# wenz116/lang2seg

Hardware: AMD Instinct MI355X
Metric: train images/sec (cycle loss on), 600×1000 input, at 1/2/4/8 MI355X (higher is better)
Workload: dtype bf16; 1 GPU; train_cycle.sh step: ResNet-101 C4 + 7 spatial dynamic filters + att2in2 cycle loss, 600x1000 image, 20-token expression (V=3349), 12000->2000 proposals, 256 RoIs, per-GPU batch 1; variant=cycle, parallelism=dp1

## Files before the change

### lang2seg_amd/csrc/roi.hip

```cpp
#include "common.h"
#include "roi_sample.h"
#include "../../include/lang2seg_hip.h"

namespace {

__global__ void rpn_decode_kernel(const float* __restrict__ heads, int ldh, const float* __restrict__ base, int H, int W, int A,
                                  int fs, float im_h, float im_w, float* prob, float* boxes, float* scores) {
  const int n = H * W * A;
  for (int i = blockIdx.x * blockDim.x + threadIdx.x; i < n; i += gridDim.x * blockDim.x) {
    const int a = i % A, pix = i / A, w = pix % W, h = pix / W;
    const float* hr = heads + (long)pix * ldh;
    const float bg = hr[a], fg = hr[A + a];
    const float m = fmaxf(bg, fg);
    const float e0 = expf(bg - m), e1 = expf(fg - m);
    const float s = e0 + e1;
    prob[(long)pix * 2 * A + a] = e0 / s;
    prob[(long)pix * 2 * A + A + a] = e1 / s;
    scores[i] = e1 / s;
    const float ax1 = base[a * 4 + 0] + (float)(w * fs), ay1 = base[a * 4 + 1] + (float)(h * fs);
    const float ax2 = base[a * 4 + 2] + (float)(w * fs), ay2 = base[a * 4 + 3] + (float)(h * fs);
    const float aw = ax2 - ax1 + 1.0f, ah = ay2 - ay1 + 1.0f;
    const float cx = ax1 + 0.5f * aw, cy = ay1 + 0.5f * ah;
    const float* d = hr + 2 * A + a * 4;
    const float pcx = d[0] * aw + cx, pcy = d[1] * ah + cy;
    const float pw = expf(d[2]) * aw, ph = expf(d[3]) * ah;
    float x1 = pcx - 0.5f * pw, y1 = pcy - 0.5f * ph, x2 = pcx + 0.5f * pw, y2 = pcy + 0.5f * ph;
    x1 = fminf(fmaxf(x1, 0.f), im_w - 1.f); y1 = fminf(fmaxf(y1, 0.f), im_h - 1.f);
    x2 = fminf(fmaxf(x2, 0.f), im_w - 1.f); y2 = fminf(fmaxf(y2, 0.f), im_h - 1.f);
    *(float4*)(boxes + (long)i * 4) = make_float4(x1, y1, x2, y2);
  }
}

__device__ __forceinline__ uint64_t sort_key(float s, int idx) {
  uint32_t u = __float_as_uint(s);
  u = (u & 0x80000000u) ? ~u : (u | 0x80000000u);
  return ((uint64_t)u << 32) | (uint32_t)(0xFFFFFFFFu - (uint32_t)idx);
}
__device__ __forceinline__ unsigned int okey(float s) { unsigned int u = __float_as_uint(s); return (u & 0x80000000u) ? ~u : (u | 0x80000000u); }
struct RsWs { unsigned int* kA; int* iA; unsigned int* kB; int* iB; int* hist; };
__device__ __host__ __forceinline__ RsWs rs_ws(int* ws, int n) {
  RsWs w; w.kA = (unsigned int*)ws; w.iA = ws + n; w.kB = (unsigned int*)(ws + 2 * n); w.iB = ws + 3 * n; w.hist = ws + 4 * n;
  return w;
}
__global__ __launch_bounds__(256) void rs_hist0_kernel(const float* scores, int n, int nblk, int* hist) {
  __shared__ int h[256];
  const int t = threadIdx.x, b = blockIdx.x;
  h[t] = 0;
  __syncthreads();
  const int i = b * 256 + t;
  if (i < n) atomicAdd(&h[(~okey(scores[i])) & 255], 1);
  __syncthreads();
  hist[b * 256 + t] = h[t];
#pragma unroll
  for (int p = 1; p < 4; ++p) hist[(p * nblk + b) * 256 + t] = 0;
}
template <int PASS>
__global__ __launch_bounds__(256) void rs_pass_kernel(const float* __restrict__ scores, const float* __restrict__ boxes, const unsigned int* __restrict__ kin,
                                                      const int* __restrict__ iin, unsigned int* __restrict__ kout, int* __restrict__ iout, int n, int nblk,
                                                      int* __restrict__ hist, int k, float* __restrict__ sboxes, float* __restrict__ sscores, int* __restrict__ sidx) {
  __shared__ int tot[256], base[256], wcnt[4][256];
  const int t = threadIdx.x, b = blockIdx.x, lane = t & 63, wave = t >> 6;
  const int i = b * 256 + t;
  unsigned int key = 0; int idx = 0;
  const bool valid = i < n;
  if (valid) {
    if (PASS == 0) { key = ~okey(scores[i]); idx = i; } else { key = kin[i]; idx = iin[i]; }
  }
  const int d = (int)((key >> (8 * PASS)) & 255u);
  __shared__ int ptot[4][256], pbef[4][256];
  {
    const int q = t & 63, g = t >> 6;
    const int4* hp4 = (const int4*)(hist + (long)PASS * nblk * 256) + q;
    int4 tv = make_int4(0, 0, 0, 0), bv = make_int4(0, 0, 0, 0);
    for (int b0 = g; b0 < nblk; b0 += 64) {
      int4 v[16];
#pragma unroll
      for (int u = 0; u < 16; ++u) v[u] = (b0 + 4 * u < nblk) ? hp4[(long)(b0 + 4 * u) * 64] : make_int4(0, 0, 0, 0);
#pragma unroll
      for (int u = 0; u < 16; ++u) {
        tv.x += v[u].x; tv.y += v[u].y; tv.z += v[u].z; tv.w += v[u].w;
        if (b0 + 4 * u < b) { bv.x += v[u].x; bv.y += v[u].y; bv.z += v[u].z; bv.w += v[u].w; }
      }
    }
    *(int4*)&ptot[g][4 * q] = tv; *(int4*)&pbef[g][4 * q] = bv;
  }
  __syncthreads();
  const int total = ptot[0][t] + ptot[1][t] + ptot[2][t] + ptot[3][t];
  const int before = pbef[0][t] + pbef[1][t] + pbef[2][t] + pbef[3][t];
#pragma unroll
  for (int w = 0; w < 4; ++w) wcnt[w][t] = 0;
  int incl = total;
#pragma unroll
  for (int o = 1; o < 64; o <<= 1) { const int x = __shfl_up(incl, o); if (lane >= o) incl += x; }
  if (lane == 63) tot[wave] = incl;
  __syncthreads();
  for (int w = 0; w < wave; ++w) incl += tot[w];
  base[t] = incl - total + before;
  unsigned long long same = valid ? ~0ull : 0ull;
#pragma unroll
  for (int bit = 0; bit < 8; ++bit) {
    const unsigned long long bal = __ballot(valid && ((d >> bit) & 1));
    same &= ((d >> bit) & 1) ? bal : ~bal;
  }
  same &= __ballot(valid);
  const int below = __popcll(same & ((1ull << lane) - 1ull));
  if (valid && below == 0) wcnt[wave][d] = __popcll(same);
  __syncthreads();
  if (valid) {
    int rank = below;
    for (int w = 0; w < wave; ++w) rank += wcnt[w][d];
    const int pos = base[d] + rank;
    if (PASS < 3) {
      kout[pos] = key; iout[pos] = idx;
      atomicAdd(&hist[((long)(PASS + 1) * nblk + (pos >> 8)) * 256 + ((key >> (8 * (PASS + 1))) & 255u)], 1);
    } else if (pos < k) {
      sidx[pos] = idx; sscores[pos] = scores[idx];
      *(float4*)(sboxes + (long)pos * 4) = *(const float4*)(boxes + (long)idx * 4);
    }
  }
}

__device__ __forceinline__ bool nms_hit(const float4& a, float aarea, const float4& b, float barea, float thr, int cmp) {
  const float xx1 = fmaxf(a.x, b.x), yy1 = fmaxf(a.y, b.y), xx2 = fminf(a.z, b.z), yy2 = fminf(a.w, b.w);
  const float w = fmaxf(0.f, xx2 - xx1 + 1.f), h = fmaxf(0.f, yy2 - yy1 + 1.f);
  const float inter = w * h;
  const float uni = aarea + barea - inter;
  const float q = thr * uni;
  if (inter < q * (1.f - 0x1p-18f)) return false;
  if (inter > q * (1.f + 0x1p-18f)) return true;
  const float ovr = inter / uni;
  return cmp ? (ovr > thr) : (ovr >= thr);
}
#ifdef L2S_TOOLS
__device__ long long nms_dbg[16];
#define NMS_T() ((long long)__builtin_readcyclecounter())
#else
#define NMS_T() 0ll
#endif
constexpr int NMS_SB = 64;
constexpr int NMS_LAG = 6;
constexpr int NMS_RING = 16;
constexpr int NMS_SLOT = NMS_LAG + 2;
__global__ __launch_bounds__(256) void nms_mask_kernel(const float* __restrict__ boxes, int n, float thr, int cmp, int row0, int sbw, uint64_t* mask,
                                                       unsigned long long* carry_base, const int* __restrict__ keep, const int* nk_p, int max_keep,
                                                       unsigned long long* carry_all, int carry_words) {
  const int wv = threadIdx.x >> 6, lane = threadIdx.x & 63;
  const int cbk = blockIdx.x * 4 + wv;
  int nk = 0;
  if (row0 > 0) { nk = *nk_p; if (nk < 0 || nk >= max_keep) return; }
  else if (blockIdx.x == 0 && blockIdx.y == 0) for (int i = threadIdx.x; i < carry_words; i += 256) carry_all[i] = 0ull;
  const bool diag = (int)blockIdx.y < sbw;
  const int rb = blockIdx.y;
  const bool active = cbk < sbw && (diag ? cbk <= rb : ((int)blockIdx.y - sbw) * 64 < nk);
  __shared__ float4 cbox_s[4][64];
  __shared__ float carea_s[4][64];
  float4* cbox = cbox_s[wv]; float* carea = carea_s[wv];
  const int cj = row0 + cbk * 64 + lane;
  const float4 cbv = (active && cj < n) ? *(const float4*)(boxes + (long)cj * 4) : make_float4(0, 0, -1, -1);
  cbox[lane] = cbv;
  carea[lane] = (cbv.z - cbv.x + 1.f) * (cbv.w - cbv.y + 1.f);
  __syncthreads();
  if (!active) return;
  unsigned long long* carry = carry_base;
  const int csize = min(64, n - row0 - cbk * 64);
  if (diag) {
    const int ri = row0 + rb * 64 + lane;
    if (ri >= n) return;
    const float4 a = *(const float4*)(boxes + (long)ri * 4);
    const float aarea = (a.z - a.x + 1.f) * (a.w - a.y + 1.f);
    uint64_t t = 0;
    if (rb == cbk) {
      for (int j = 0; j < lane; ++j)
        if (nms_hit(cbox[j], carea[j], a, aarea, thr, cmp)) t |= 1ull << j;
    } else {
      for (int j = 0; j < 64; ++j)
        if (nms_hit(cbox[j], carea[j], a, aarea, thr, cmp)) t |= 1ull << j;
    }
    mask[(long)(rb * sbw + cbk) * 64 + lane] = t;
    return;
  }
  const int ki = ((int)blockIdx.y - sbw) * 64 + lane;
  uint64_t t = 0;
  if (ki < nk) {
    const int ri = keep[ki];
    const float4 a = *(const float4*)(boxes + (long)ri * 4);
    const float aarea = (a.z - a.x + 1.f) * (a.w - a.y + 1.f);
    for (int j = 0; j < csize; ++j)
      if (nms_hit(a, aarea, cbox[j], carea[j], thr, cmp)) t |= 1ull << j;
  }
  unsigned int lo = (unsigned int)t, hi = (unsigned int)(t >> 32);
#pragma unroll
  for (int off = 32; off; off >>= 1) { lo |= __shfl_xor(lo, off); hi |= __shfl_xor(hi, off); }
  if (lane == 0 && (lo | hi)) atomicOr(&carry[cbk], ((unsigned long long)hi << 32) | lo);
}
__global__ __launch_bounds__(1024) void nms_reduce_kernel(const uint64_t* __restrict__ mask, int n, int cb, int max_keep, int* keep, int* num_out,
                                                          int row0, const unsigned long long* __restrict__ carry) {
  constexpr int LAG = NMS_LAG, SLOT = NMS_SLOT, NBULK = 15;
  extern __shared__ unsigned long long slots[];
  __shared__ int kdone_sh, stop_sh;
  __shared__ int ready_sh[NMS_SB];
  unsigned long long* ksh = slots + (size_t)NMS_RING * SLOT * 64;
  unsigned long long* csh = ksh + cb;
  const int tid = threadIdx.x, lane = tid & 63, wave = __builtin_amdgcn_readfirstlane(tid >> 6);
  int nk0 = 0;
  if (row0 > 0) { nk0 = *num_out; if (nk0 < 0 || nk0 >= max_keep) return; }
  for (int c = tid; c < cb; c += 1024) { ksh[c] = 0ull; csh[c] = carry ? carry[c] : 0ull; ready_sh[c] = 0; }
  if (tid == 0) { kdone_sh = 0; stop_sh = 0; }
  __syncthreads();
  typedef __attribute__((address_space(3))) volatile int lds_vint;
  typedef __attribute__((address_space(3))) volatile unsigned long long lds_vu64;
  auto lds_ld = [](const int* p) { const int v = *(const lds_vint*)p; asm volatile("" ::: "memory"); return v; };
  auto lds_st = [](int* p, int v) { asm volatile("" ::: "memory"); *(lds_vint*)p = v; };
  auto lds_ld64 = [](const unsigned long long* p) { return *(const lds_vu64*)p; };
  auto lds_st64 = [](unsigned long long* p, unsigned long long v) { *(lds_vu64*)p = v; };
  auto poll = [&](int* p, int want) {
    int spins = 0;
    while (lds_ld(p) < want) {
      __builtin_amdgcn_s_sleep(1);
      if (++spins > (1 << 22)) { *(volatile int*)num_out = -1; __builtin_amdgcn_endpgm(); }
    }
  };
  if (wave == 0) {
    __builtin_amdgcn_s_setprio(3);
    int nk = nk0;
    unsigned long long kprev[LAG];
#pragma unroll
    for (int k = 0; k < LAG; ++k) kprev[k] = 0ull;
    long long t_wait = 0, t_res = 0; const long long t_begin = NMS_T(); int nb_done = 0;
    for (int b = 0; b < cb; ++b) {
      const long long tp = NMS_T();
      poll(&ready_sh[b], 1);
      const long long tr = NMS_T();
      t_wait += tr - tp; ++nb_done;
      const unsigned long long* sl = slots + (size_t)(b % NMS_RING) * SLOT * 64 + lane;
      unsigned long long hit = sl[0];
#pragma unroll
      for (int k = 1; k <= LAG; ++k) hit |= sl[k * 64] & kprev[LAG - k];
      const unsigned long long d = sl[(LAG + 1) * 64];
      unsigned long long rb = __ballot(hit != 0ull) | csh[b];
      const int lim = min(64, n - b * 64);
      if (lim < 64) rb |= ~0ull << lim;
      const unsigned long long alive = ~rb;
      unsigned long long kept = alive;
      for (int sweep = 0; sweep < 65; ++sweep) {
        const unsigned long long nk2 = alive & ~__ballot((d & kept) != 0ull);
        if (nk2 == kept) break;
        kept = nk2;
      }
      rb = ~kept;
      const unsigned long long K = ~rb;
      if (lane == 0) {
        lds_st64(&ksh[b], K);
        lds_st(&kdone_sh, b + 1);
      }
      t_res += NMS_T() - tr;
      const int row = b * 64 + lane;
      if ((K >> lane) & 1ull) { const int pos = nk + __popcll(K & ((1ull << lane) - 1ull)); if (pos < max_keep) keep[pos] = row0 + row; }
      nk += __popcll(K);
#pragma unroll
      for (int k = LAG - 1; k > 0; --k) kprev[k] = kprev[k - 1];
      kprev[0] = K;
      if (nk >= max_keep) break;
    }
    if (lane == 0) {
#ifdef L2S_TOOLS
      nms_dbg[0] = NMS_T() - t_begin; nms_dbg[1] = t_wait; nms_dbg[2] = nb_done; nms_dbg[7] = t_res;
#endif
      lds_st(&stop_sh, 1);
      lds_st(&kdone_sh, 1 << 20);
      *num_out = min(nk, max_keep);
    }
    return;
  }
  long long t_ld = 0, t_k = 0, t_tail = 0; const long long t_begin = NMS_T();
  for (int b = wave - 1; b < cb; b += NBULK) {
    if (lds_ld(&stop_sh)) break;
    const uint64_t* tb = mask + (long)b * cb * 64 + lane;
    unsigned long long* sl = slots + (size_t)(b % NMS_RING) * SLOT * 64 + lane;
    const int nold = b - LAG;
    unsigned long long acc = 0ull;
    unsigned long long raw[LAG + 1];
#pragma unroll
    for (int k = 0; k <= LAG; ++k) raw[k] = tb[(long)max(nold + k, 0) * 64];
    for (int base = 0; base < nold; base += 32) {
      unsigned long long tw[32];
      const long long tl = NMS_T();
#pragma unroll
      for (int i = 0; i < 32; ++i) tw[i] = tb[(long)min(base + i, b) * 64];
#pragma unroll
      for (int i = 0; i < 32; ++i) asm volatile("" : "+v"(tw[i]));
      t_ld += NMS_T() - tl;
      const int hi = min(nold, base + 32);
      int from = base;
      for (int pass = 0; pass < 2 && from < hi; ++pass) {
        int have = __builtin_amdgcn_readfirstlane(lds_ld(&kdone_sh));
        if (pass == 1) {
          const long long tk = NMS_T();
          int spins = 0;
          while (have < hi) {
            __builtin_amdgcn_s_sleep(1);
            if (++spins > (1 << 22)) { *(volatile int*)num_out = -1; __builtin_amdgcn_endpgm(); }
            have = __builtin_amdgcn_readfirstlane(lds_ld(&kdone_sh));
          }
          t_k += NMS_T() - tk;
        }
        const int to = min(have, hi);
        const unsigned long long kw = (lane < 32 && base + lane >= from && base + lane < to) ? lds_ld64(&ksh[base + lane]) : 0ull;
        const unsigned int klo = (unsigned int)kw, khi = (unsigned int)(kw >> 32);
#pragma unroll
        for (int i = 0; i < 32; ++i) {
          const unsigned int k0 = __builtin_amdgcn_readlane(klo, i), k1 = __builtin_amdgcn_readlane(khi, i);
          acc |= tw[i] & (((unsigned long long)k1 << 32) | k0);
        }
        from = to;
      }
    }
    const long long tt = NMS_T();
#pragma unroll
    for (int k = 0; k < LAG; ++k) sl[(k + 1) * 64] = nold + k >= 0 ? raw[k] : 0ull;
    sl[(LAG + 1) * 64] = raw[LAG];
    t_tail += NMS_T() - tt;
    lds_st64(&sl[0], acc);
    lds_st(&ready_sh[b], 1);
  }
#ifdef L2S_TOOLS
  if (wave == 1 && lane == 0) { nms_dbg[3] = t_ld; nms_dbg[4] = t_k; nms_dbg[5] = NMS_T() - t_begin; nms_dbg[6] = t_tail; }
#endif
}
__global__ void gather_rois_kernel(const float* sboxes, const float* sscores, const int* keep, const int* num, int max_keep, float* rois, float* rs) {
  const int i = blockIdx.x * blockDim.x + threadIdx.x;
  if (i >= max_keep) return;
  float4 b = make_float4(0, 0, 0, 0); float sc = 0.f;
  if (i < *num) { int k = keep[i]; b = *(const float4*)(sboxes + (long)k * 4); sc = sscores[k]; }
  rois[i * 5 + 0] = 0.f; rois[i * 5 + 1] = b.x; rois[i * 5 + 2] = b.y; rois[i * 5 + 3] = b.z; rois[i * 5 + 4] = b.w;
  rs[i] = sc;
}

struct AtlWs { int* cnt; unsigned long long* gtmax; double* maxov; int* argmax; int* lab; };
__device__ __forceinline__ AtlWs atl_ws(int* ws, int n) {
  AtlWs w;
  w.cnt = ws; w.gtmax = (unsigned long long*)(ws + 16); w.maxov = (double*)(ws + 16 + 64);
  w.argmax = ws + 16 + 64 + 2 * n; w.lab = w.argmax + n;
  return w;
}
__device__ __forceinline__ void anchor_at(const float* base, int i, int A, int W, int fs, float& x1, float& y1, float& x2, float& y2) {
  const int a = i % A, pix = i / A, w = pix % W, h = pix / W;
  x1 = base[a * 4 + 0] + (float)(w * fs); y1 = base[a * 4 + 1] + (float)(h * fs);
  x2 = base[a * 4 + 2] + (float)(w * fs); y2 = base[a * 4 + 3] + (float)(h * fs);
}
__device__ __forceinline__ double iou64(float ax1, float ay1, float ax2, float ay2, const float* g) {
  const double bx1 = ax1, by1 = ay1, bx2 = ax2, by2 = ay2, qx1 = g[0], qy1 = g[1], qx2 = g[2], qy2 = g[3];
  const double ba = (bx2 - bx1 + 1) * (by2 - by1 + 1), qa = (qx2 - qx1 + 1) * (qy2 - qy1 + 1);
  double iw = fmin(bx2, qx2) - fmax(bx1, qx1) + 1; if (iw < 0) iw = 0;
  double ih = fmin(by2, qy2) - fmax(by1, qy1) + 1; if (ih < 0) ih = 0;
  return iw * ih / (ba + qa - iw * ih);
}
__global__ void atl_init_kernel(int* ws) { if (threadIdx.x < 16 + 64) ws[threadIdx.x] = 0; }
__global__ void atl_iou_kernel(const float* gt, int n_gt, const float* base, int n, int W, int A, int fs, float im_h, float im_w, int* ws) {
  AtlWs w = atl_ws(ws, n);
  const int i = blockIdx.x * blockDim.x + threadIdx.x;
  if (i >= n) return;
  float x1, y1, x2, y2; anchor_at(base, i, A, W, fs, x1, y1, x2, y2);
  const bool inside = x1 >= 0.f && y1 >= 0.f && x2 < im_w && y2 < im_h;
  double best = -1.0; int arg = 0;
  if (inside) {
    for (int g = 0; g < n_gt; ++g) {
      double o = iou64(x1, y1, x2, y2, gt + g * 5);
      if (o > best) { best = o; arg = g; }
      atomicMax(&w.gtmax[g], (unsigned long long)__double_as_longlong(o));
    }
  }
  w.maxov[i] = best; w.argmax[i] = arg;
  w.lab[i] = inside ? -1 : -2;
}
__global__ void atl_label_kernel(const float* gt, int n_gt, const float* base, int n, int W, int A, int fs, float neg_ov, float pos_ov, int* ws) {
  AtlWs w = atl_ws(ws, n);
  const int i = blockIdx.x * blockDim.x + threadIdx.x;
  const bool live = i < n && w.lab[min(i, n - 1)] != -2;
  int l = -1;
  if (live) {
    float x1, y1, x2, y2; anchor_at(base, i, A, W, fs, x1, y1, x2, y2);
    const double mo = w.maxov[i];
    if (mo < (double)neg_ov) l = 0;
    for (int g = 0; g < n_gt; ++g)
      if (iou64(x1, y1, x2, y2, gt + g * 5) == __longlong_as_double((long long)w.gtmax[g])) l = 1;
    if (mo >= (double)pos_ov) l = 1;
    w.lab[i] = l;
  }
  const unsigned long long m1 = __ballot(l == 1), m0 = __ballot(l == 0);
  if ((threadIdx.x & 63) == (unsigned)__builtin_ctzll(__ballot(1))) {
    if (m1) atomicAdd(&w.cnt[0], __popcll(m1));
    if (m0) atomicAdd(&w.cnt[1], __popcll(m0));
  }
}
__device__ void select_disable(int* lab, const uint32_t* keys, int n, int which, int D, int* hist , int* sh ) {
  const int tid = threadIdx.x;
  if (D <= 0) return;
  uint32_t prefix = 0, pmask = 0; int need = D;
  for (int pass = 3; pass >= 0; --pass) {
    for (int b = tid; b < 256; b += blockDim.x) hist[b] = 0;
    __syncthreads();
    for (int i = tid; i < n; i += blockDim.x)
      if (lab[i] == which && (keys[i] & pmask) == prefix) atomicAdd(&hist[(keys[i] >> (8 * pass)) & 255], 1);
    __syncthreads();
    if (tid == 0) {
      int acc = 0, b = 0;
      for (; b < 256; ++b) { if (acc + hist[b] >= need) break; acc += hist[b]; }
      sh[0] = b; sh[1] = need - acc;
    }
    __syncthreads();
    prefix |= ((uint32_t)sh[0]) << (8 * pass); pmask |= 255u << (8 * pass); need = sh[1];
    __syncthreads();
  }
  if (tid == 0) sh[2] = 0;
  __syncthreads();
  for (int i0 = 0; i0 < n; i0 += blockDim.x) {
    const int i = i0 + tid;
    bool cand = i < n && lab[i] == which;
    if (cand && keys[i] < prefix) { lab[i] = -1; cand = false; }
    const bool tie = cand && keys[i] == prefix;
    if (tie) { int tk = atomicAdd(&sh[2], 1); if (tk < need) lab[i] = -1; }
    __syncthreads();
  }
}
__device__ __forceinline__ void select_disable_lds(signed char* lab, const uint32_t* key, int n, int which, int D, int* hist , int* sh ) {
  const int tid = threadIdx.x;
  if (D <= 0) return;
  uint32_t prefix = 0, pmask = 0; int need = D;
  for (int pass = 3; pass >= 0; --pass) {
    if (tid < 256) hist[tid] = 0;
    __syncthreads();
#pragma unroll 4
    for (int i = tid; i < n; i += 1024) {
      const uint32_t k = key[i];
      if (lab[i] == which && (k & pmask) == prefix) atomicAdd(&hist[(k >> (8 * pass)) & 255], 1);
    }
    __syncthreads();
    if (tid < 64) {
      const int c0 = hist[4 * tid], c1 = hist[4 * tid + 1], c2 = hist[4 * tid + 2], c3 = hist[4 * tid + 3];
      const int tot = c0 + c1 + c2 + c3;
      int inc = tot;
#pragma unroll
      for (int o = 1; o < 64; o <<= 1) { const int v = __shfl_up(inc, o, 64); if (tid >= o) inc += v; }
      const int before = inc - tot;
      if (before < need && inc >= need) {
        int acc = before, b = 4 * tid;
        if (acc + c0 < need) { acc += c0; ++b; if (acc + c1 < need) { acc += c1; ++b; if (acc + c2 < need) { acc += c2; ++b; } } }
        sh[0] = b; sh[1] = need - acc;
      }
    }
    __syncthreads();
    prefix |= ((uint32_t)sh[0]) << (8 * pass); pmask |= 255u << (8 * pass); need = sh[1];
    __syncthreads();
  }
  if (tid == 0) sh[2] = 0;
  __syncthreads();
  int nt = 0;
#pragma unroll 4
  for (int i = tid; i < n; i += 1024) {
    const uint32_t k = key[i];
    const bool c = lab[i] == which;
    if (c && k < prefix) lab[i] = -1;
    nt += (c && k == prefix);
  }
  if (nt) atomicAdd(&sh[2], nt);
  __syncthreads();
  const int nties = sh[2];
  if (nties == need) {
#pragma unroll 4
    for (int i = tid; i < n; i += 1024) if (lab[i] == which && key[i] == prefix) lab[i] = -1;
  } else {
    int left = need;
    for (int i0 = 0; i0 < n && left > 0; i0 += 1024) {
      const int i = i0 + tid;
      const bool tie = i < n && lab[i] == which && key[i] == prefix;
      const unsigned long long bm = __ballot(tie);
// ... 269 lines not shown
          const double sx = (double)cw / (double)ms, sy = (double)ch / (double)ms;
          double xo = 0.5 * sx, yo = 0.5 * sy;
          for (int k = 0; k < px; ++k) xo += sx;
          for (int k = 0; k < py; ++k) yo += sy;
          const int ix = min((int)xo, cw - 1), iy = min((int)yo, ch - 1);
          addr[q] = ((long)g6[4] * im_h + (g6[1] + iy)) * im_w + (g6[0] + ix);
          val[q] = true;
        }
      }
    }
    uint8_t m[4];
#pragma unroll
    for (int q = 0; q < 4; ++q) m[q] = val[q] ? gt_masks[addr[q]] : (uint8_t)0;
#pragma unroll
    for (int q = 0; q < 4; ++q) { const int e = e0 + q * nt; if (e < total) mt[e] = (float)m[q]; }
  }
}

__global__ void roialign_fwd_kernel(const void* feat, int H, int W, int C, const float* rois, int P, float sscale, float TH, float TW, void* out, int dt) {
  const int cell = blockIdx.x, r = cell / (P * P), rem = cell - r * P * P, py = rem / P, px = rem - py * P;
  const Samp s = roi_sample(rois + r * 5, H, W, P, py, px, sscale, TH, TW);
  const float w00 = (1.f - s.wx1) * (1.f - s.wy1), w01 = s.wx1 * (1.f - s.wy1), w10 = (1.f - s.wx1) * s.wy1, w11 = s.wx1 * s.wy1;
  const bool vx0 = s.x0 >= 0 && s.x0 < W, vx1 = s.x0 + 1 >= 0 && s.x0 + 1 < W, vy0 = s.y0 >= 0 && s.y0 < H, vy1 = s.y0 + 1 >= 0 && s.y0 + 1 < H;
  for (int c = threadIdx.x; c < C; c += blockDim.x) {
    float v = 0.f;
    if (vy0 && vx0) v += w00 * ldx(feat, ((long)s.y0 * W + s.x0) * C + c, dt);
    if (vy0 && vx1) v += w01 * ldx(feat, ((long)s.y0 * W + s.x0 + 1) * C + c, dt);
    if (vy1 && vx0) v += w10 * ldx(feat, ((long)(s.y0 + 1) * W + s.x0) * C + c, dt);
    if (vy1 && vx1) v += w11 * ldx(feat, ((long)(s.y0 + 1) * W + s.x0 + 1) * C + c, dt);
    stx(out, (long)cell * C + c, dt, v);
  }
}
__global__ __launch_bounds__(128) void roialign_fwd_bf16x8_kernel(const bf16_t* __restrict__ feat, int H, int W, int C, const float* __restrict__ rois, int P,
                                                                 float sscale, float TH, float TW, bf16_t* out) {
  const int cell = blockIdx.x, r = cell / (P * P), rem = cell - r * P * P, py = rem / P, px = rem - py * P;
  const RoiTaps t = roi_taps(roi_sample(rois + r * 5, H, W, P, py, px, sscale, TH, TW), H, W, C);
  for (int c = threadIdx.x * 8; c < C; c += blockDim.x * 8) *(uint4*)(out + (long)cell * C + c) = roi_blend8(feat, t, c);
}
__global__ void roialign_bwd_kernel(const void* dout, int H, int W, int C, const float* rois, int P, float sscale, float TH, float TW, float* dfeat, int dt) {
  const int cell = blockIdx.x, r = cell / (P * P), rem = cell - r * P * P, py = rem / P, px = rem - py * P;
  const Samp s = roi_sample(rois + r * 5, H, W, P, py, px, sscale, TH, TW);
  const float w00 = (1.f - s.wx1) * (1.f - s.wy1), w01 = s.wx1 * (1.f - s.wy1), w10 = (1.f - s.wx1) * s.wy1, w11 = s.wx1 * s.wy1;
  const bool vx0 = s.x0 >= 0 && s.x0 < W, vx1 = s.x0 + 1 >= 0 && s.x0 + 1 < W, vy0 = s.y0 >= 0 && s.y0 < H, vy1 = s.y0 + 1 >= 0 && s.y0 + 1 < H;
  for (int c = threadIdx.x; c < C; c += blockDim.x) {
    const float g = ldx(dout, (long)cell * C + c, dt);
    if (vy0 && vx0) atomicAdd(dfeat + ((long)s.y0 * W + s.x0) * C + c, w00 * g);
    if (vy0 && vx1) atomicAdd(dfeat + ((long)s.y0 * W + s.x0 + 1) * C + c, w01 * g);
    if (vy1 && vx0) atomicAdd(dfeat + ((long)(s.y0 + 1) * W + s.x0) * C + c, w10 * g);
    if (vy1 && vx1) atomicAdd(dfeat + ((long)(s.y0 + 1) * W + s.x0 + 1) * C + c, w11 * g);
  }
}


__device__ __forceinline__ void ra_load4(const float* p, float v[4]) {
  const float4 q = *(const float4*)p; v[0] = q.x; v[1] = q.y; v[2] = q.z; v[3] = q.w;
}
__device__ __forceinline__ void ra_load4(const bf16_t* p, float v[4]) {
  const uint2 q = *(const uint2*)p;
  v[0] = __uint_as_float(q.x << 16); v[1] = __uint_as_float(q.x & 0xffff0000u);
  v[2] = __uint_as_float(q.y << 16); v[3] = __uint_as_float(q.y & 0xffff0000u);
}
template <typename T>
__global__ __launch_bounds__(256) void roialign_bwd_gather_kernel(const T* dout, int H, int W, int C, const float* rois, int R, int P,
                                                                  float sscale, float TH, float TW, float* dfeat) {
  constexpr int CAP = 2048;
  __shared__ int e_cell[CAP];
  __shared__ float e_w[CAP];
  __shared__ int sc[256];
  const int pix = blockIdx.x, y = pix / W, x = pix - y * W, t = threadIdx.x, nv = C >> 2;
  bool wrote = false;
  for (int r0 = 0; r0 < R; r0 += 256) {
    const int r = r0 + t;
    unsigned my = 0, mx = 0;
    if (r < R) {
      for (int i = 0; i < P; ++i) {
        const Samp s = roi_sample(rois + r * 5, H, W, P, i, i, sscale, TH, TW);
        const float wyv = (s.y0 == y ? 1.f - s.wy1 : 0.f) + (s.y0 + 1 == y ? s.wy1 : 0.f);
        const float wxv = (s.x0 == x ? 1.f - s.wx1 : 0.f) + (s.x0 + 1 == x ? s.wx1 : 0.f);
        if (wyv != 0.f) my |= 1u << i;
        if (wxv != 0.f) mx |= 1u << i;
      }
    }
    const int n = __popc(my) * __popc(mx);
    sc[t] = n;
    __syncthreads();
    for (int o = 1; o < 256; o <<= 1) {
      const int v = t >= o ? sc[t - o] : 0;
      __syncthreads();
      sc[t] += v;
      __syncthreads();
    }
    const int total = sc[255], off = sc[t] - n;
    __syncthreads();
    for (int wb = 0; wb < total; wb += CAP) {
      if (n && off < wb + CAP && off + n > wb) {
        int k = off;
        for (unsigned a = my; a; a &= a - 1) {
          const int py = __ffs(a) - 1;
          for (unsigned b = mx; b; b &= b - 1, ++k) {
            if (k < wb || k >= wb + CAP) continue;
            const int px = __ffs(b) - 1;
            const Samp s = roi_sample(rois + r * 5, H, W, P, py, px, sscale, TH, TW);
            const float wyv = s.y0 == y ? 1.f - s.wy1 : s.wy1, wxv = s.x0 == x ? 1.f - s.wx1 : s.wx1;
            e_cell[k - wb] = (r * P + py) * P + px;
            e_w[k - wb] = wxv * wyv;
          }
        }
      }
      __syncthreads();
      const int ne = min(CAP, total - wb);
      for (int v = t; v < nv; v += 256) {
        float a0 = 0.f, a1 = 0.f, a2 = 0.f, a3 = 0.f;
        const T* base = dout + v * 4;
#pragma unroll 4
        for (int e = 0; e < ne; ++e) {
          float g[4];
          ra_load4(base + (long)e_cell[e] * C, g);
          const float w = e_w[e];
          a0 += w * g[0]; a1 += w * g[1]; a2 += w * g[2]; a3 += w * g[3];
        }
        float4* d = (float4*)(dfeat + (long)pix * C + v * 4);
        float4 q = wrote ? *d : make_float4(0.f, 0.f, 0.f, 0.f); q.x += a0; q.y += a1; q.z += a2; q.w += a3; *d = q;
      }
      wrote = true;
      __syncthreads();
    }
  }
  if (!wrote)
    for (int v = t; v < nv; v += 256) *(float4*)(dfeat + (long)pix * C + v * 4) = make_float4(0.f, 0.f, 0.f, 0.f);
}

}

extern "C" int l2s_rpn_decode(const float* heads, int ldh, const float* base_anchors, int H, int W, int A, int feat_stride,
                              float im_h, float im_w, float* prob, float* boxes, float* scores, hipStream_t s) {
  const int n = H * W * A;
  L2S_LAUNCH(rpn_decode_kernel, dim3(cdiv(n, 256)), dim3(256), 0, s, heads, ldh, base_anchors, H, W, A, feat_stride, im_h, im_w, prob, boxes, scores);
  return l2s_check_launch();
}
extern "C" long l2s_sort_ws_ints(int n) { return 4L * n + 4L * 256L * cdiv(n, 256) + 64; }
extern "C" int l2s_sort_topk(const float* scores, const float* boxes, int n, int k, int* ws, float* sorted_boxes,
                             float* sorted_scores, int* sorted_idx, hipStream_t s) {
  if (!ws || n <= 0 || k > n) return L2S_EINVAL;
  const int nblk = cdiv(n, 256);
  RsWs w = rs_ws(ws, n);
  L2S_LAUNCH(rs_hist0_kernel, dim3(nblk), dim3(256), 0, s, scores, n, nblk, w.hist);
  L2S_LAUNCH(rs_pass_kernel<0>, dim3(nblk), dim3(256), 0, s, scores, boxes, (const unsigned int*)nullptr, (const int*)nullptr, w.kA, w.iA, n, nblk, w.hist, k, sorted_boxes, sorted_scores, sorted_idx);
  L2S_LAUNCH(rs_pass_kernel<1>, dim3(nblk), dim3(256), 0, s, scores, boxes, (const unsigned int*)w.kA, (const int*)w.iA, w.kB, w.iB, n, nblk, w.hist, k, sorted_boxes, sorted_scores, sorted_idx);
  L2S_LAUNCH(rs_pass_kernel<2>, dim3(nblk), dim3(256), 0, s, scores, boxes, (const unsigned int*)w.kB, (const int*)w.iB, w.kA, w.iA, n, nblk, w.hist, k, sorted_boxes, sorted_scores, sorted_idx);
  L2S_LAUNCH(rs_pass_kernel<3>, dim3(nblk), dim3(256), 0, s, scores, boxes, (const unsigned int*)w.kA, (const int*)w.iA, w.kB, w.iB, n, nblk, w.hist, k, sorted_boxes, sorted_scores, sorted_idx);
  return l2s_check_launch();
}
static inline size_t nms_mask_words(int n) { const int sbw = min(cdiv(n, 64), NMS_SB); return (size_t)sbw * sbw * 64; }
static inline size_t nms_scan_lds(int sbw) { return ((size_t)NMS_RING * NMS_SLOT * 64 + 2 * (size_t)sbw) * 8; }
extern "C" size_t l2s_nms_workspace_bytes(int n) { return (nms_mask_words(n) + (size_t)cdiv(cdiv(n, 64), NMS_SB) * NMS_SB) * 8; }
extern "C" int l2s_nms(const float* sorted_boxes, int n, float thresh, int cmp_mode, int max_keep, uint64_t* mask_ws,
                       int* keep_out, int* num_out, hipStream_t s) {
  if (n <= 0 || max_keep < 1) return L2S_EINVAL;
  const int cb = cdiv(n, 64), nst = cdiv(cb, NMS_SB);
  static bool attr_done = false;
  if (!attr_done) { (void)hipFuncSetAttribute((const void*)nms_reduce_kernel, hipFuncAttributeMaxDynamicSharedMemorySize, (int)nms_scan_lds(NMS_SB)); attr_done = true; }
  unsigned long long* carry_all = (unsigned long long*)mask_ws + nms_mask_words(n);
  for (int st = 0; st < nst; ++st) {
    const int row0 = st * NMS_SB * 64, rows = min(n - row0, NMS_SB * 64), sbw = cdiv(rows, 64);
    unsigned long long* carry = carry_all + (size_t)st * NMS_SB;
    L2S_LAUNCH(nms_mask_kernel, dim3(cdiv(sbw, 4), sbw + (st ? cdiv(max_keep, 64) : 0)), dim3(256), 0, s, sorted_boxes, n, thresh, cmp_mode, row0, sbw, mask_ws,
               carry, (const int*)keep_out, (const int*)num_out, max_keep, carry_all, nst * NMS_SB);
    L2S_LAUNCH(nms_reduce_kernel, dim3(1), dim3(1024), nms_scan_lds(sbw), s, (const uint64_t*)mask_ws, rows, sbw, max_keep, keep_out, num_out, row0,
               st ? (const unsigned long long*)carry : (const unsigned long long*)nullptr);
  }
  return l2s_check_launch();
}
#ifdef L2S_TOOLS
extern "C" int l2s_tools_nms_dbg(long long* host16) { return hipMemcpyFromSymbol(host16, HIP_SYMBOL(nms_dbg), sizeof(long long) * 16) == hipSuccess ? 0 : L2S_ELAUNCH; }
#endif
extern "C" int l2s_gather_rois(const float* sorted_boxes, const float* sorted_scores, const int* keep, const int* num, int max_keep,
                               float* rois, float* roi_scores, hipStream_t s) {
  L2S_LAUNCH(gather_rois_kernel, dim3(cdiv(max_keep, 256)), dim3(256), 0, s, sorted_boxes, sorted_scores, keep, num, max_keep, rois, roi_scores);
  return l2s_check_launch();
}
extern "C" const int* l2s_anchor_target_count(const int* ws) { return ws + 2; }
extern "C" long l2s_anchor_target_ws_ints(int hwa) { return 16 + 64 + 4L * hwa + 16; }
extern "C" int l2s_anchor_target(const float* gt, int n_gt, const float* base_anchors, int H, int W, int A, int feat_stride,
                                 float im_h, float im_w, const uint32_t* fg_keys, const uint32_t* bg_keys,
                                 float neg_ov, float pos_ov, int batch, float fg_frac,
                                 int* labels, float* targets, float* inside_w, float* outside_w, int* ws, hipStream_t s) {
  if (n_gt < 1 || n_gt > 32) return L2S_EINVAL;
  const int n = H * W * A;
  L2S_LAUNCH(atl_init_kernel, dim3(1), dim3(128), 0, s, ws);
  L2S_LAUNCH(atl_iou_kernel, dim3(cdiv(n, 256)), dim3(256), 0, s, gt, n_gt, base_anchors, n, W, A, feat_stride, im_h, im_w, ws);
  L2S_LAUNCH(atl_label_kernel, dim3(cdiv(n, 256)), dim3(256), 0, s, gt, n_gt, base_anchors, n, W, A, feat_stride, neg_ov, pos_ov, ws);
  if (n <= ATL_LDS_MAX) {
    static bool attr_done = false;
    if (!attr_done) { (void)hipFuncSetAttribute((const void*)atl_sample_lds_kernel, hipFuncAttributeMaxDynamicSharedMemorySize, (256 + 24) * 4 + ATL_LDS_MAX * 5); attr_done = true; }
    const int npad = (n + 3) / 4 * 4;
    L2S_LAUNCH(atl_sample_lds_kernel, dim3(1), dim3(1024), (size_t)(256 + 24) * 4 + (size_t)npad * 5, s, fg_keys, bg_keys, n, npad, batch, fg_frac, ws);
  } else {
    L2S_LAUNCH(atl_sample_kernel, dim3(1), dim3(1024), 0, s, fg_keys, bg_keys, n, batch, fg_frac, ws);
  }
  L2S_LAUNCH(atl_out_kernel, dim3(cdiv(n, 256)), dim3(256), 0, s, gt, base_anchors, n, H, W, A, feat_stride, (const int*)ws, labels, targets, inside_w, outside_w);
  return l2s_check_launch();
}
extern "C" int l2s_proposal_target(const float* rois, const float* roi_scores, const int* n_rois, int n_max, const float* gt, int n_gt,
                                   const uint8_t* gt_masks, int im_h, int im_w, const uint32_t* fg_keys, const uint32_t* bg_keys,
                                   const uint32_t* bg_rand, int R, int fg_max, int mask_slots, float fg_thresh, float bg_hi, float bg_lo,
                                   const float* means4, const float* stds4, const float* inw4, int ncls, int ms,
                                   float* out_rois, int* labels, float* bbox_targets, float* bbox_inside, float* bbox_outside,
                                   float* mask_targets, int* counts, int* ws, hipStream_t s) {
  if (n_gt < 1 || R < 1 || mask_slots < 1 || mask_slots > R || mask_slots * 6 > 8192) return L2S_EINVAL;
  const size_t tb = (size_t)R * 4 * ncls * sizeof(float);
  if ((char*)bbox_inside == (char*)bbox_targets + tb && (char*)bbox_outside == (char*)bbox_inside + tb) {
    if (l2s_memset_async(bbox_targets, 0, 3 * tb, s)) return L2S_ELAUNCH;
  } else if (l2s_memset_async(bbox_targets, 0, tb, s) || l2s_memset_async(bbox_inside, 0, tb, s) || l2s_memset_async(bbox_outside, 0, tb, s)) return L2S_ELAUNCH;
  L2S_LAUNCH(ptl_kernel, dim3(1), dim3(1024), 0, s, rois, roi_scores, n_rois, n_max, gt, n_gt, gt_masks, im_h, im_w,
                     fg_keys, bg_keys, bg_rand, R, fg_max, mask_slots, fg_thresh, bg_hi, bg_lo, means4, stds4, inw4, ncls, ms,
                     out_rois, labels, bbox_targets, bbox_inside, bbox_outside, mask_targets, counts, ws);
  return l2s_check_launch();
}
static int roialign_fwd_launch(const void* feat, int H, int W, int C, const float* rois, int R, int P, float sscale, float TH, float TW,
                               void* out, int dtype, hipStream_t s) {
  if (dtype == L2S_BF16 && !(C & 7) && !((uintptr_t)feat & 15) && !((uintptr_t)out & 15)) {
    L2S_LAUNCH(roialign_fwd_bf16x8_kernel, dim3(R * P * P), dim3(C >= 1024 ? 128 : 64), 0, s, (const bf16_t*)feat, H, W, C, rois, P, sscale, TH, TW, (bf16_t*)out);
    return l2s_check_launch();
  }
  L2S_LAUNCH(roialign_fwd_kernel, dim3(R * P * P), dim3(256), 0, s, feat, H, W, C, rois, P, sscale, TH, TW, out, dtype);
  return l2s_check_launch();
}
static int roialign_bwd_launch(const void* dout, int H, int W, int C, const float* rois, int R, int P, float sscale, float TH, float TW,
                               float* dfeat, int dtype, hipStream_t s) {
  if (C % 4 == 0 && P <= 32) {
    if (dtype) L2S_LAUNCH(roialign_bwd_gather_kernel<bf16_t>, dim3(H * W), dim3(256), 0, s, (const bf16_t*)dout, H, W, C, rois, R, P, sscale, TH, TW, dfeat);
    else L2S_LAUNCH(roialign_bwd_gather_kernel<float>, dim3(H * W), dim3(256), 0, s, (const float*)dout, H, W, C, rois, R, P, sscale, TH, TW, dfeat);
    return l2s_check_launch();
  }
  if (l2s_memset_async(dfeat, 0, (size_t)H * W * C * sizeof(float), s)) return L2S_ELAUNCH;
  L2S_LAUNCH(roialign_bwd_kernel, dim3(R * P * P), dim3(256), 0, s, dout, H, W, C, rois, P, sscale, TH, TW, dfeat, dtype);
  return l2s_check_launch();
}
extern "C" int l2s_roialign_fwd(const void* feat, int H, int W, int C, const float* rois, int R, int P, float spatial_scale,
                                void* out, int dtype, hipStream_t s) {
  return roialign_fwd_launch(feat, H, W, C, rois, R, P, spatial_scale, (float)H, (float)W, out, dtype, s);
}
extern "C" int l2s_roialign_bwd(const void* dout, int H, int W, int C, const float* rois, int R, int P, float spatial_scale,
                                float* dfeat, int dtype, hipStream_t s) {
  return roialign_bwd_launch(dout, H, W, C, rois, R, P, spatial_scale, (float)H, (float)W, dfeat, dtype, s);
}
extern "C" int l2s_cropalign_fwd(const void* feat, int H, int W, int C, const float* rois, int R, int P, float im_h, float im_w,
                                 void* out, int dtype, hipStream_t s) {
  return roialign_fwd_launch(feat, H, W, C, rois, R, P, 1.f, im_h, im_w, out, dtype, s);
}
extern "C" int l2s_cropalign_bwd(const void* dout, int H, int W, int C, const float* rois, int R, int P, float im_h, float im_w,
                                 float* dfeat, int dtype, hipStream_t s) {
  return roialign_bwd_launch(dout, H, W, C, rois, R, P, 1.f, im_h, im_w, dfeat, dtype, s);
}
extern "C" int l2s_roipool_fwd(const void* feat, int H, int W, int C, const float* rois, int R, int P, float spatial_scale, void* out,
                               int* argmax, int dtype, hipStream_t s) {
  L2S_LAUNCH(roipool_fwd_kernel, dim3(R * P * P), dim3(256), 0, s, feat, H, W, C, rois, P, spatial_scale, out, argmax, dtype);
  return l2s_check_launch();
}
extern "C" int l2s_roipool_bwd(const void* dout, const int* argmax, int R, int P, int C, float* dfeat, int dtype, hipStream_t s) {
  const long n = (long)R * P * P * C;
  long g = (n + 255) / 256; if (g > 8192) g = 8192;
  L2S_LAUNCH(roipool_bwd_kernel, dim3((int)g), dim3(256), 0, s, dout, argmax, n, C, dfeat, dtype);
  return l2s_check_launch();
}
```

Before: 225.7 img/s.

## Resolve NMS column blocks in pairs to halve serial scan iterations

The NMS reduce kernel's serial wave now resolves two 64-box column blocks per step instead of one. Bulk waves precompute the accumulated suppression for both blocks of each pair, plus the cross-block mask, so the resolver runs one joint fixed-point sweep over both. The intent is to halve the number of serial poll/resolve iterations on the critical path of this single-block kernel. In exchange each bulk wave does more loads and the ring and batch sizes shrink, and the joint sweep loop can take more iterations.

```diff
diff --git a/lang2seg_amd/csrc/roi.hip b/lang2seg_amd/csrc/roi.hip
--- a/lang2seg_amd/csrc/roi.hip
+++ b/lang2seg_amd/csrc/roi.hip
@@ -138,9 +138,10 @@
 #define NMS_T() 0ll
 #endif
 constexpr int NMS_SB = 64;
-constexpr int NMS_LAG = 6;
-constexpr int NMS_RING = 16;
-constexpr int NMS_SLOT = NMS_LAG + 2;
+constexpr int NMS_LAG = 3;
+constexpr int NMS_LAGB = 2 * NMS_LAG;
+constexpr int NMS_RING = 8;
+constexpr int NMS_SLOT = 2 + 2 * NMS_LAGB + 3;
 __global__ __launch_bounds__(256) void nms_mask_kernel(const float* __restrict__ boxes, int n, float thr, int cmp, int row0, int sbw, uint64_t* mask,
                                                        unsigned long long* carry_base, const int* __restrict__ keep, const int* nk_p, int max_keep,
                                                        unsigned long long* carry_all, int carry_words) {
@@ -195,16 +196,19 @@
 }
 __global__ __launch_bounds__(1024) void nms_reduce_kernel(const uint64_t* __restrict__ mask, int n, int cb, int max_keep, int* keep, int* num_out,
                                                           int row0, const unsigned long long* __restrict__ carry) {
-  constexpr int LAG = NMS_LAG, SLOT = NMS_SLOT, NBULK = 15;
+  constexpr int LAGB = NMS_LAGB, SLOT = NMS_SLOT, NBULK = 15, BATCH = 16;
+  constexpr int S_RA = 2, S_RB = 2 + LAGB, S_DA = 2 + 2 * LAGB, S_XB = S_DA + 1, S_DB = S_DA + 2;
   extern __shared__ unsigned long long slots[];
   __shared__ int kdone_sh, stop_sh;
-  __shared__ int ready_sh[NMS_SB];
+  __shared__ int ready_sh[NMS_SB / 2];
+  const int np = (cb + 1) >> 1;
   unsigned long long* ksh = slots + (size_t)NMS_RING * SLOT * 64;
-  unsigned long long* csh = ksh + cb;
+  unsigned long long* csh = ksh + 2 * np;
   const int tid = threadIdx.x, lane = tid & 63, wave = __builtin_amdgcn_readfirstlane(tid >> 6);
   int nk0 = 0;
   if (row0 > 0) { nk0 = *num_out; if (nk0 < 0 || nk0 >= max_keep) return; }
-  for (int c = tid; c < cb; c += 1024) { ksh[c] = 0ull; csh[c] = carry ? carry[c] : 0ull; ready_sh[c] = 0; }
+  for (int c = tid; c < 2 * np; c += 1024) { ksh[c] = 0ull; csh[c] = (carry && c < cb) ? carry[c] : 0ull; }
+  for (int c = tid; c < np; c += 1024) ready_sh[c] = 0;
   if (tid == 0) { kdone_sh = 0; stop_sh = 0; }
   __syncthreads();
   typedef __attribute__((address_space(3))) volatile int lds_vint;
@@ -223,43 +227,49 @@
   if (wave == 0) {
     __builtin_amdgcn_s_setprio(3);
     int nk = nk0;
-    unsigned long long kprev[LAG];
-#pragma unroll
-    for (int k = 0; k < LAG; ++k) kprev[k] = 0ull;
+    unsigned long long kprev[LAGB];
+#pragma unroll
+    for (int k = 0; k < LAGB; ++k) kprev[k] = 0ull;
     long long t_wait = 0, t_res = 0; const long long t_begin = NMS_T(); int nb_done = 0;
-    for (int b = 0; b < cb; ++b) {
+    for (int p = 0; p < np; ++p) {
       const long long tp = NMS_T();
-      poll(&ready_sh[b], 1);
+      poll(&ready_sh[p], 1);
       const long long tr = NMS_T();
       t_wait += tr - tp; ++nb_done;
-      const unsigned long long* sl = slots + (size_t)(b % NMS_RING) * SLOT * 64 + lane;
-      unsigned long long hit = sl[0];
-#pragma unroll
-      for (int k = 1; k <= LAG; ++k) hit |= sl[k * 64] & kprev[LAG - k];
-      const unsigned long long d = sl[(LAG + 1) * 64];
-      unsigned long long rb = __ballot(hit != 0ull) | csh[b];
-      const int lim = min(64, n - b * 64);
-      if (lim < 64) rb |= ~0ull << lim;
-      const unsigned long long alive = ~rb;
-      unsigned long long kept = alive;
-      for (int sweep = 0; sweep < 65; ++sweep) {
-        const unsigned long long nk2 = alive & ~__ballot((d & kept) != 0ull);
-        if (nk2 == kept) break;
-        kept = nk2;
-      }
-      rb = ~kept;
-      const unsigned long long K = ~rb;
+      const unsigned long long* sl = slots + (size_t)(p % NMS_RING) * SLOT * 64 + lane;
+      unsigned long long hitA = sl[0], hitB = sl[64];
+#pragma unroll
+      for (int k = 0; k < LAGB; ++k) {
+        hitA |= sl[(S_RA + k) * 64] & kprev[LAGB - 1 - k];
+        hitB |= sl[(S_RB + k) * 64] & kprev[LAGB - 1 - k];
+      }
+      const unsigned long long dA = sl[S_DA * 64], xB = sl[S_XB * 64], dB = sl[S_DB * 64];
+      unsigned long long rA = __ballot(hitA != 0ull) | csh[2 * p], rB = __ballot(hitB != 0ull) | csh[2 * p + 1];
+      const int limA = n - p * 128, limB = limA - 64;
+      if (limA < 64) rA |= ~0ull << limA;
+      if (limB < 64) rB |= limB > 0 ? ~0ull << limB : ~0ull;
+      const unsigned long long aliveA = ~rA, aliveB = ~rB;
+      unsigned long long KA = aliveA, KB = aliveB;
+      for (int sweep = 0; sweep < 129; ++sweep) {
+        const unsigned long long nA = aliveA & ~__ballot((dA & KA) != 0ull);
+        const unsigned long long nB = aliveB & ~__ballot(((dB & KB) | (xB & KA)) != 0ull);
+        if (nA == KA && nB == KB) break;
+        KA = nA; KB = nB;
+      }
       if (lane == 0) {
-        lds_st64(&ksh[b], K);
-        lds_st(&kdone_sh, b + 1);
+        lds_st64(&ksh[2 * p], KA);
+        lds_st64(&ksh[2 * p + 1], KB);
+        lds_st(&kdone_sh, 2 * p + 2);
       }
       t_res += NMS_T() - tr;
-      const int row = b * 64 + lane;
-      if ((K >> lane) & 1ull) { const int pos = nk + __popcll(K & ((1ull << lane) - 1ull)); if (pos < max_keep) keep[pos] = row0 + row; }
-      nk += __popcll(K);
-#pragma unroll
-      for (int k = LAG - 1; k > 0; --k) kprev[k] = kprev[k - 1];
-      kprev[0] = K;
+      const unsigned long long below = (1ull << lane) - 1ull;
+      const int nkB = nk + __popcll(KA);
+      if ((KA >> lane) & 1ull) { const int pos = nk + __popcll(KA & below); if (pos < max_keep) keep[pos] = row0 + p * 128 + lane; }
+      if ((KB >> lane) & 1ull) { const int pos = nkB + __popcll(KB & below); if (pos < max_keep) keep[pos] = row0 + p * 128 + 64 + lane; }
+      nk = nkB + __popcll(KB);
+#pragma unroll
+      for (int k = LAGB - 1; k > 1; --k) kprev[k] = kprev[k - 2];
+      kprev[1] = KA; kprev[0] = KB;
       if (nk >= max_keep) break;
     }
     if (lane == 0) {
@@ -273,24 +283,29 @@
     return;
   }
   long long t_ld = 0, t_k = 0, t_tail = 0; const long long t_begin = NMS_T();
-  for (int b = wave - 1; b < cb; b += NBULK) {
+  for (int p = wave - 1; p < np; p += NBULK) {
     if (lds_ld(&stop_sh)) break;
-    const uint64_t* tb = mask + (long)b * cb * 64 + lane;
-    unsigned long long* sl = slots + (size_t)(b % NMS_RING) * SLOT * 64 + lane;
-    const int nold = b - LAG;
-    unsigned long long acc = 0ull;
-    unsigned long long raw[LAG + 1];
-#pragma unroll
-    for (int k = 0; k <= LAG; ++k) raw[k] = tb[(long)max(nold + k, 0) * 64];
-    for (int base = 0; base < nold; base += 32) {
-      unsigned long long tw[32];
+    const int ba = 2 * p, bb = min(ba + 1, cb - 1);
+    const bool hasB = ba + 1 < cb;
+    const uint64_t* ta = mask + (long)ba * cb * 64 + lane;
+    const uint64_t* tb = mask + (long)bb * cb * 64 + lane;
+    unsigned long long* sl = slots + (size_t)(p % NMS_RING) * SLOT * 64 + lane;
+    const int nold = ba - LAGB;
+    unsigned long long accA = 0ull, accB = 0ull;
+    unsigned long long rawA[LAGB + 1], rawB[LAGB + 2];
+#pragma unroll
+    for (int k = 0; k <= LAGB; ++k) rawA[k] = ta[(long)max(nold + k, 0) * 64];
+#pragma unroll
+    for (int k = 0; k <= LAGB + 1; ++k) rawB[k] = tb[(long)min(max(nold + k, 0), bb) * 64];
+    for (int base = 0; base < nold; base += BATCH) {
+      unsigned long long twA[BATCH], twB[BATCH];
       const long long tl = NMS_T();
 #pragma unroll
-      for (int i = 0; i < 32; ++i) tw[i] = tb[(long)min(base + i, b) * 64];
-#pragma unroll
-      for (int i = 0; i < 32; ++i) asm volatile("" : "+v"(tw[i]));
+      for (int i = 0; i < BATCH; ++i) { const long c = min(base + i, ba); twA[i] = ta[c * 64]; twB[i] = tb[c * 64]; }
+#pragma unroll
+      for (int i = 0; i < BATCH; ++i) asm volatile("" : "+v"(twA[i]), "+v"(twB[i]));
       t_ld += NMS_T() - tl;
-      const int hi = min(nold, base + 32);
+      const int hi = min(nold, base + BATCH);
       int from = base;
       for (int pass = 0; pass < 2 && from < hi; ++pass) {
         int have = __builtin_amdgcn_readfirstlane(lds_ld(&kdone_sh));
@@ -305,23 +320,30 @@
           t_k += NMS_T() - tk;
         }
         const int to = min(have, hi);
-        const unsigned long long kw = (lane < 32 && base + lane >= from && base + lane < to) ? lds_ld64(&ksh[base + lane]) : 0ull;
+        const unsigned long long kw = (lane < BATCH && base + lane >= from && base + lane < to) ? lds_ld64(&ksh[base + lane]) : 0ull;
         const unsigned int klo = (unsigned int)kw, khi = (unsigned int)(kw >> 32);
 #pragma unroll
-        for (int i = 0; i < 32; ++i) {
+        for (int i = 0; i < BATCH; ++i) {
           const unsigned int k0 = __builtin_amdgcn_readlane(klo, i), k1 = __builtin_amdgcn_readlane(khi, i);
-          acc |= tw[i] & (((unsigned long long)k1 << 32) | k0);
+          const unsigned long long kk = ((unsigned long long)k1 << 32) | k0;
+          accA |= twA[i] & kk; accB |= twB[i] & kk;
         }
         from = to;
       }
     }
     const long long tt = NMS_T();
 #pragma unroll
-    for (int k = 0; k < LAG; ++k) sl[(k + 1) * 64] = nold + k >= 0 ? raw[k] : 0ull;
-    sl[(LAG + 1) * 64] = raw[LAG];
+    for (int k = 0; k < LAGB; ++k) {
+      sl[(S_RA + k) * 64] = nold + k >= 0 ? rawA[k] : 0ull;
+      sl[(S_RB + k) * 64] = hasB && nold + k >= 0 ? rawB[k] : 0ull;
+    }
+    sl[S_DA * 64] = rawA[LAGB];
+    sl[S_XB * 64] = hasB ? rawB[LAGB] : 0ull;
+    sl[S_DB * 64] = hasB ? rawB[LAGB + 1] : 0ull;
     t_tail += NMS_T() - tt;
-    lds_st64(&sl[0], acc);
-    lds_st(&ready_sh[b], 1);
+    lds_st64(&sl[64], hasB ? accB : 0ull);
+    lds_st64(&sl[0], accA);
+    lds_st(&ready_sh[p], 1);
   }
 #ifdef L2S_TOOLS
   if (wave == 1 && lane == 0) { nms_dbg[3] = t_ld; nms_dbg[4] = t_k; nms_dbg[5] = NMS_T() - t_begin; nms_dbg[6] = t_tail; }
@@ -897,7 +919,7 @@
   return l2s_check_launch();
 }
 static inline size_t nms_mask_words(int n) { const int sbw = min(cdiv(n, 64), NMS_SB); return (size_t)sbw * sbw * 64; }
-static inline size_t nms_scan_lds(int sbw) { return ((size_t)NMS_RING * NMS_SLOT * 64 + 2 * (size_t)sbw) * 8; }
+static inline size_t nms_scan_lds(int sbw) { return ((size_t)NMS_RING * NMS_SLOT * 64 + 4 * (size_t)cdiv(sbw, 2)) * 8; }
 extern "C" size_t l2s_nms_workspace_bytes(int n) { return (nms_mask_words(n) + (size_t)cdiv(cdiv(n, 64), NMS_SB) * NMS_SB) * 8; }
 extern "C" int l2s_nms(const float* sorted_boxes, int n, float thresh, int cmp_mode, int max_keep, uint64_t* mask_ws,
                        int* keep_out, int* num_out, hipStream_t s) {
```

Result: no change. 226.1 img/s, median of 4 (+0.2%).
